# ray-project/kuberay

Measured on NVIDIA H100. Metric: reconciles/sec over 10k RayCluster x 100 pods (batched reconcilePods + status roll-up), higher is better.
Workload: dtype u32

## Files before the change

kuberay_b200/csrc/kr_bucket2.cuh:

```cuda
#pragma once

#include "kr_decide.cuh"

namespace kr {

__device__ __forceinline__ uint32_t inc_epoch_of(const ScratchDev &sc) { return __ldcg(&sc.inc[KR_INC_EPOCH]) + 1u; }

#ifndef KR_D2WARPS
#define KR_D2WARPS 8
#endif
static constexpr int kD2Warps = KR_D2WARPS;
#define KR_ROW_UNHEALTHY (1u << 13)
#define KR_ROW_FRESH (1u << 14)
#define KR_LG_OWNED (1u << 31)

__device__ __forceinline__ uint4 *large_slot(const ScratchDev &sc, uint32_t c, uint32_t rank) {
  if (!sc.lg) return nullptr;
  const uint4 l = __ldcg(&sc.lg[c]);
  const uint32_t j = rank - sc.bucket_stride;
  return j < l.y ? sc.region + l.x + j : nullptr;
}
__device__ __forceinline__ uint4 *rec_slot(const ScratchDev &sc, uint32_t c, uint32_t rank) {
  return rank < sc.bucket_stride ? sc.bucket + (size_t)c * sc.bucket_stride + rank : large_slot(sc, c, rank);
}


template <int kItems>
__global__ void __launch_bounds__(kSortThreads) k_match2(SnapDev s, ScratchDev sc, ResDev r, Sizes n, int has_wtd) {
  KR_TL(1);
  extern __shared__ uint32_t sm_bits[];
  __shared__ uint32_t s_orph[kSortThreads / 32];
  const uint32_t tile = blockIdx.x;
  const uint32_t warp = threadIdx.x >> 5, lane = threadIdx.x & 31;
  const uint32_t base = tile * (kSortThreads * kItems) + warp * (32 * kItems) + lane;
  uint32_t ns[kItems], cn[kItems], gn[kItems], nm[kItems], pk[kItems], ri[kItems];
#pragma unroll
  for (int it = 0; it < kItems; it++) {
    const uint32_t p = base + it * 32;
    const bool v = p < n.n_pods;
    ns[it] = v ? __ldg(&s.p_ns_id[p]) : 0u; cn[it] = v ? __ldg(&s.p_cluster_name_id[p]) : 0u;
    gn[it] = v ? __ldg(&s.p_group_name_id[p]) : 0u; nm[it] = v ? __ldg(&s.p_name_id[p]) : 0u;
    pk[it] = v ? __ldg(&s.p_packed[p]) : 0u; ri[it] = v ? (uint32_t)__ldg(&s.p_replica_index[p]) : 0u;
  }
  pdl_wait(); pdl_trigger();
  uint32_t pi[kItems];
  uint4 sl[kItems];
#pragma unroll
  for (int it = 0; it < kItems; it++) {
    pi[it] = hash_pair(ns[it], cn[it]) & sc.cl_mask;
    sl[it] = __ldg(&sc.cl_slots[pi[it]]);
  }
  if (has_wtd) {
    const uint32_t words = (sc.wt_bits_mask + 1) >> 5;
    for (uint32_t i = threadIdx.x; i < words; i += kSortThreads) sm_bits[i] = __ldcg(&sc.wt_bits[i]);
    __syncthreads();
  }
  uint32_t orphans = 0;
  uint32_t cidx[kItems], roww[kItems];
#pragma unroll
  for (int it = 0; it < kItems; it++) {
    const uint32_t p = base + it * 32;
    const bool v = p < n.n_pods;
    uint32_t c = n.n_clusters, cflags = 0, gname0 = 0;
    if (cn[it] != 0) {
      uint4 q = sl[it];
      uint32_t i = pi[it];
      while (true) {
        if (q.x == cn[it] && q.y == ns[it]) { c = q.w >> 2; cflags = q.w & 3u; gname0 = q.z; break; }
        if (q.x == KR_EMPTY32 && q.y == KR_EMPTY32) break;
        i = (i + 1) & sc.cl_mask;
        q = __ldg(&sc.cl_slots[i]);
      }
    }
    const bool matched = v && c < n.n_clusters;
    uint32_t slot = KR_ROW_NO_GROUP, g0 = 0xFFFFFFFFu;
    if (matched && gn[it] != 0) {
      if (gname0 == gn[it]) slot = 0;
      else if (cflags & KR_CL_MULTI) {
        const uint4 rec = __ldg(&sc.cl_rec[c]);
        g0 = rec.x;
        for (uint32_t gi = 1; gi < rec.y; gi++)
          if (__ldg(&s.g_name_id[g0 + gi]) == gn[it]) { slot = gi; break; }
      }
    }
    uint32_t flags = pk[it] & (0x7FFu | KR_PP_TOMBSTONE);
    if (should_delete(pk[it])) flags |= KR_ROW_UNHEALTHY;
    if (has_wtd && v) {
      const uint32_t hk = hash_pair(ns[it], nm[it]);
      const uint32_t h2 = bloom2(hk);
      if ((sm_bits[(hk & sc.wt_bits_mask) >> 5] & (1u << (hk & 31))) && (sm_bits[(h2 & sc.wt_bits_mask) >> 5] & (1u << (h2 & 31)))) {
        const uint64_t k = key2(ns[it], nm[it]);
        uint32_t i = hk & sc.wt_mask;
        uint64_t kk = __ldg(&sc.wt_keys[i]);
        while (kk != KR_EMPTY64) {
          if (kk == k) {
            for (uint32_t e = sc.wt_head[i]; e != KR_EMPTY32; e = sc.wt_next[e]) {
// ... 139 lines not shown
      if ((((labelled | noname) >> k) & 1u) && (pw[k] & KR_ROW_WTD_OWN)) {
        const uint32_t r = ((noname >> k) & 1u) ? r_empty : rep[k];
        if (r != KR_MH_NONE) atomicOr(&s_rep[r], KR_MHF_WTD);
      }
    }
    __syncwarp();
    int32_t n_del = 0;
#pragma unroll
    for (int k = 0; k < K; k++) {
      const bool hit = ((labelled >> k) & 1u) && (s_rep[rep[k]] & KR_MHF_WTD);
      if (hit && act[k] == KR_ACT_KEEP) act[k] = KR_ACT_DELETE_MH_WTD;
      n_del += __popc(__ballot_sync(0xFFFFFFFFu, hit));
    }
    gr.flags |= KR_GR_WTD_EXECUTED;
    if (n_del > 0) { gr.flags |= KR_GR_ABORTED; err_arg = n_del; return KR_ERR_MH_WTD; }
  }
  int32_t running = 0;
  for (uint32_t r = lane; r < n_rep; r += 32) running += (s_rep[r] & KR_MHF_DELETED) ? 0 : 1;
  running = __reduce_add_sync(0xFFFFFFFFu, running);
#pragma unroll
  for (int k = 0; k < K; k++) if (((heads >> k) & 1u) && !(s_rep[rep[k]] & KR_MHF_DELETED)) mh_head |= 1u << k;
  gr.n_running = running;
  if (expected % H != 0) { gr.flags |= KR_GR_ABORTED; err_arg = expected; return KR_ERR_MH_NOT_MULTIPLE; }
  const int32_t to_create = expected / H - running;
  gr.diff = to_create;
  if (to_create > 0) gr.n_create = (uint32_t)to_create;
  else if (to_create < 0) {
    if (delete_allowed) {
      const int32_t remove = -to_create;
      int32_t seen = 0;
      for (uint32_t b = 0; b < n_rep && seen < remove; b += 32) {
        const uint32_t r = b + lane;
        const bool ok = r < n_rep && !(s_rep[r] & KR_MHF_DELETED);
        const uint32_t bal = __ballot_sync(0xFFFFFFFFu, ok);
        if (ok && seen + (int32_t)__popc(bal & lt) < remove) s_rep[r] |= KR_MHF_SCALE;
        seen += __popc(bal);
      }
      __syncwarp();
#pragma unroll
      for (int k = 0; k < K; k++) if (((labelled >> k) & 1u) && (s_rep[rep[k]] & KR_MHF_SCALE)) act[k] = KR_ACT_DELETE_MH_SCALE_DOWN;
    } else gr.flags |= KR_GR_RANDOM_DELETE_OFF;
  }
  return KR_ERR_NONE;
}

template <int K, bool kInc = false, bool kMH = false>
__global__ void __launch_bounds__(kD2Warps * 32, (K <= 4 && !kMH ? 32 : 16) / kD2Warps) k_decide2(Decide2Args a) {
  const int phase = kInc ? 2 : a.phase;
  KR_TL(phase ? 12 : 3);
  __shared__ int32_t s_acc[kD2Warps][3][KR_SMEM_GROUPS];
  __shared__ int32_t s_mode[kD2Warps][kMH ? 4 : 3][KR_SMEM_GROUPS];
  __shared__ uint32_t s_list[kD2Warps][32 * K];
  __shared__ uint32_t s_bits[kD2Warps][32];
  const SnapDev &s = a.s;
  const uint32_t warp = threadIdx.x >> 5, lane = threadIdx.x & 31;
  const uint32_t lt = lanemask_lt();
  const uint32_t S = a.sc.bucket_stride;
  uint32_t c = blockIdx.x * kD2Warps + warp;
  bool mine = phase == 0 && c < a.n.n_clusters;
  RecordCI ci{mine ? __ldg(&a.sc.cl_in[32 * (size_t)c + lane]) : 0u};
  pdl_wait(); pdl_trigger();
  if (phase == 1) {
    mine = c < a.r.totals[4];
    if (mine) { c = a.sc.deferred_list[c]; ci.word = __ldg(&a.sc.cl_in[32 * (size_t)c + lane]); }
  } else if (kInc) {
    mine = c < __ldcg(&a.sc.inc[KR_INC_DIRTY]) && !__ldcg(&a.sc.inc[KR_INC_VOID]) && !__ldcg(&a.sc.inc[KR_INC_STRUCTURAL]);
    if (mine) {
      c = a.sc.dirty_list[c];
      ci.word = __ldcg(&a.sc.cl_in[32 * (size_t)c + lane]);
    }
  }
  if (KR_ATTEMPT_VOID(a.r.totals)) mine = false;
  if (ci.group_cnt() > KR_SMEM_GROUPS) mine = false;
  if (kInc && !mine) return;
  uint4 *bucket = a.sc.bucket + (size_t)(mine ? c : 0) * S;
  uint4 dyn = make_uint4(0, 0, 0, 0);
  uint4 recs[K] = {};
  if (mine) {
    dyn = __ldcg(&a.sc.cl_dyn[c]);
#pragma unroll
    for (int k = 0; k < K; k++) if ((uint32_t)(k * 32) + lane < S) recs[k] = __ldcg(&bucket[k * 32 + lane]);
  }
  uint32_t P = dyn.x;
  if (P > S) { mine = false; P = 0; }
  if (kInc) {
    const uint32_t epoch = inc_epoch_of(a.sc);
    const bool lost = dyn.y == epoch;
    uint32_t kept = 0, head_min = 0xFFFFFFFFu;
#pragma unroll
    for (int k = 0; k < K; k++) {
      const uint32_t j = k * 32 + lane;
      bool keep = mine && j < P;
      const bool fresh = keep && (recs[k].y & KR_ROW_FRESH);
      if (keep && lost && !fresh) keep = __ldcg(&a.sc.stamp[recs[k].x]) != epoch;
      const uint32_t bal = __ballot_sync(0xFFFFFFFFu, keep);
      if (keep) {
        uint4 rec = recs[k];
        rec.y &= ~KR_ROW_FRESH;
        const uint32_t to = kept + __popc(bal & lt);
        if (fresh || to != j) { bucket[to] = rec; if (to != j) a.sc.pos[rec.x] = to; }
        if (pp_node_type(rec.y & 0xFFFFu) == KR_NT_HEAD) head_min = min(head_min, rec.x);
      }
      kept += __popc(bal);
    }
    head_min = __reduce_min_sync(0xFFFFFFFFu, head_min);
    __syncwarp();
    unsigned long long raw = 0;
    if (mine) {
      if (lane == 0 && head_min != 0xFFFFFFFFu) raw = ~(((unsigned long long)head_min << 32) | (uint32_t)(aux_lookup(a.sc, head_min) + 1));
      raw = __shfl_sync(0xFFFFFFFFu, raw, 0);
      P = kept;
      dyn = make_uint4(kept, 0u, (uint32_t)raw, (uint32_t)(raw >> 32));
      if (lane == 0) a.sc.cl_dyn[c] = dyn;
#pragma unroll
      for (int k = 0; k < K; k++) if ((uint32_t)(k * 32) + lane < kept) recs[k] = __ldcg(&bucket[k * 32 + lane]);
    }
  }
  const uint32_t cf = ci.flags(), G = ci.group_cnt(), g0 = ci.group_off();
  const uint8_t suspend_status = ci.suspend_status(), ext_err = ci.ext_err_kind(), old_prov = ci.cond_status(KR_COND_PROVISIONED);
  const bool gate = a.f.gate_status_conditions != 0;
  uint32_t old_create = 0;
  if (kInc && mine) {
    for (uint32_t gi = lane; gi < G; gi += 32) old_create += a.r.groups[g0 + gi].n_create;
    old_create = __reduce_add_sync(0xFFFFFFFFu, old_create);
  }
  uint32_t head_pod = 0xFFFFFFFFu;
  int32_t head_aux = -1;
  {
    const unsigned long long raw = ((unsigned long long)dyn.w << 32) | dyn.z;
    if (mine && raw != 0) { const unsigned long long key = ~raw; head_pod = (uint32_t)(key >> 32); head_aux = (int32_t)(uint32_t)key - 1; }
  }
  uint8_t h_ver = KR_VER_EMPTY, h_ast = KR_ANNOT_EMPTY;
  if (head_aux >= 0 && (cf & KR_CF_UPGRADE_RECREATE)) { h_ver = s.h_version_state[head_aux]; h_ast = s.h_annot_state[head_aux]; }
  uint32_t pidx[K], pw[K], ridx[K], act[K];
  uint32_t head_pos = 0xFFFFFFFFu, head_name = 0, head_flags = 0;
#pragma unroll
  for (int k = 0; k < K; k++) {
    const uint32_t i = k * 32 + lane;
    const bool valid = i < P;
    pidx[k] = valid ? recs[k].x : 0xFFFFFFFFu; pw[k] = valid ? recs[k].y : (KR_ROW_NO_GROUP << 16); ridx[k] = valid ? recs[k].z : 0u; act[k] = KR_ACT_KEEP;
    const uint32_t hit = __ballot_sync(0xFFFFFFFFu, valid && recs[k].x == head_pod);
    if (hit) {
      const int src = __ffs(hit) - 1;
      head_pos = k * 32 + src;
      head_name = __shfl_sync(0xFFFFFFFFu, recs[k].w, src); head_flags = __shfl_sync(0xFFFFFFFFu, recs[k].y, src) & 0xFFFFu;
    }
  }
  (void)head_pos;
  int32_t *acc_list = s_acc[warp][0], *acc_unh = s_acc[warp][1], *acc_wtd = s_acc[warp][2];
  int32_t *g_mode = s_mode[warp][0], *g_prefix = s_mode[warp][1], *g_ncreate = s_mode[warp][2], *g_mh_running = s_mode[warp][kMH ? 3 : 2];
  uint32_t mh_head = 0;
  if (lane < KR_SMEM_GROUPS) { acc_list[lane] = 0; acc_unh[lane] = 0; acc_wtd[lane] = 0; g_mode[lane] = GM_UNPROCESSED; g_prefix[lane] = 0; g_ncreate[lane] = 0; }
  __syncwarp();

  int32_t ready = 0, available = 0, n_heads = 0, n0_list = 0, n0_unh = 0, n0_wtd = 0;
  bool all_running = P > 0;
  const uint32_t nchunks = (P + 31) / 32;
#pragma unroll
  for (int k = 0; k < K; k++) {
    if ((uint32_t)k >= nchunks) break;
    const bool valid = (uint32_t)(k * 32) + lane < P;
    const uint32_t w = pw[k], fl = w & 0xFFFFu, slot = valid ? (w >> 16) : KR_ROW_NO_GROUP;
    const uint32_t nt = pp_node_type(fl), ph = pp_phase(fl), rd = pp_ready(fl);
    const bool w_run = valid && nt == KR_NT_WORKER && ph == KR_PHASE_RUNNING;
    available += __popc(__ballot_sync(0xFFFFFFFFu, w_run));
    ready += __popc(__ballot_sync(0xFFFFFFFFu, w_run && rd == KR_COND_TRUE));
    const bool not_ok = valid && (ph != KR_PHASE_RUNNING || rd == KR_COND_FALSE || rd == KR_COND_UNKNOWN);
    if (__any_sync(0xFFFFFFFFu, not_ok)) all_running = false;
    n_heads += __popc(__ballot_sync(0xFFFFFFFFu, valid && nt == KR_NT_HEAD));
    if (G == 1) {
      const bool in0 = slot == 0;
      n0_list += __popc(__ballot_sync(0xFFFFFFFFu, in0));
      n0_unh += __popc(__ballot_sync(0xFFFFFFFFu, in0 && (fl & KR_ROW_UNHEALTHY)));
      n0_wtd += __popc(__ballot_sync(0xFFFFFFFFu, in0 && (fl & KR_ROW_WTD_OWN)));
      continue;
    }
    const uint32_t gkey = (slot < G) ? slot : KR_ROW_NO_GROUP;
    const uint32_t peers = __match_any_sync(0xFFFFFFFFu, gkey);
    if (gkey != KR_ROW_NO_GROUP) {
      const uint32_t ub = __ballot_sync(peers, (fl & KR_ROW_UNHEALTHY) != 0);
      const uint32_t wb = __ballot_sync(peers, (fl & KR_ROW_WTD_OWN) != 0);
      if ((peers & lt) == 0) {
        acc_list[gkey] += __popc(peers);
        acc_unh[gkey] += __popc(ub & peers);
        acc_wtd[gkey] += __popc(wb & peers);
      }
    }
    __syncwarp();
  }
  if (G == 1) { if (lane == 0) { acc_list[0] = n0_list; acc_unh[0] = n0_unh; acc_wtd[0] = n0_wtd; } __syncwarp(); }

  kr_cluster_result cr;
  {
    uint32_t *z = reinterpret_cast<uint32_t *>(&cr);
#pragma unroll
    for (int k = 0; k < (int)(sizeof(cr) / 4); k++) z[k] = 0;
  }
  cr.head_pod_idx = -1; cr.stop_after_group = -1;
  uint8_t all_action = KR_ACT_KEEP;
  bool head_delete = false, run_groups = false, deferred = false, any_prefix = false;
  uint32_t n_create_cluster = 0;
  if (mine) {
    if (cf & KR_CF_SKIP) {
      cr.path = KR_PATH_SKIPPED;
    } else if (ext_err != KR_EXT_ERR_NONE) {
      cr.path = KR_PATH_SKIPPED;
      cr.err_kind = ext_err == KR_EXT_ERR_STATUS_ONLY_NIL ? KR_ERR_NONE : KR_ERR_EXTERNAL;
    } else if (suspend_status == KR_SUSPEND_SUSPENDING || (!gate && (cf & KR_CF_SUSPEND))) {
      cr.path = KR_PATH_SUSPENDING_DELETE_ALL; all_action = KR_ACT_DELETE_ALL_SUSPEND;
    } else if (gate && (suspend_status == KR_SUSPEND_SUSPENDED || (cf & KR_CF_SUSPEND))) {
      cr.path = KR_PATH_SUSPENDED_NOOP;
    } else {
      bool recreate = false;
      if ((cf & KR_CF_UPGRADE_RECREATE) && n_heads > 0) {
        const int32_t aux = head_aux;
        const uint8_t ver = h_ver, ast = h_ast;
        if (ver == KR_VER_DIFFERENT) cr.head_update_annotations = 1;
        else if (ast == KR_ANNOT_OTHER) recreate = true;
        else if (ast == KR_ANNOT_HASH32 && !a.f.skip_hash) {
          if (phase == 0 && !a.spin_hash) {
            deferred = true;
            if (lane == 0) a.sc.deferred_list[atomicAdd(&a.r.totals[4], 1u)] = c;
          } else {
            const uint8_t *ah = s.h_annot_hash + 32 * (size_t)aux;
            const uint32_t *hw = reinterpret_cast<const uint32_t *>(a.r.hash + 32 * (size_t)c);
            if (phase == 0) {
              if (lane == 0) {
                const volatile uint32_t *w7 = hw + 7;
                uint32_t it = 0;
                while (*w7 == 0u && it < 40000u) { __nanosleep(100); it++; }
                if (*w7 == 0u) atomicOr(&a.r.totals[3], KR_TOTALS_HASH_WAIT);
              }
              __syncwarp();
              __threadfence();
            }
            const uint32_t word = __ldcg(&hw[lane >> 2]);
            recreate = __any_sync(0xFFFFFFFFu, ah[lane] != (uint8_t)(word >> (8 * (lane & 3))));
          }
        }
      }
      if (recreate) {
        cr.path = KR_PATH_RECREATE_DELETE_ALL; all_action = KR_ACT_DELETE_ALL_RECREATE;
      } else {
        cr.path = KR_PATH_NORMAL;
        if (!(cf & KR_CF_HEAD_EXPECT_OK)) { cr.head_action = KR_HEAD_EXPECT_PENDING; run_groups = true; }
        else if (n_heads == 1) {
          if (head_flags & KR_ROW_UNHEALTHY) { cr.head_action = KR_HEAD_DELETE; cr.err_kind = KR_ERR_HEAD_DELETED; head_delete = true; }
          else run_groups = true;
        } else if (n_heads == 0) {
          if (old_prov == KR_COND_TRUE && (cf & KR_CF_SKIP_HEAD_RESTART)) cr.head_action = KR_HEAD_SKIP_RESTART;
          else { cr.head_action = KR_HEAD_CREATE; run_groups = true; }
// ... 21 lines not shown
        } else {
          const int32_t expected = desired_replicas(g_rep, g_mn, g_mx, hosts, gf);
          const int32_t n_list = acc_list[gi], n_unh = acc_unh[gi], n_wtd = acc_wtd[gi];
          gr.expected = expected; gr.n_list = n_list;
          if (gf & KR_GF_SUSPEND) { gr.flags |= KR_GR_SUSPENDED; mode = GM_SUSPENDED; }
          else if (kMH && hosts > 1 && a.f.gate_multihost_indexing) {
            gr.flags |= KR_GR_MULTIHOST; mode = GM_MULTIHOST;
            int32_t earg = 0;
            const int ek = decide_multihost2<K>(s, gi, expected, hosts, !autoscaling || a.f.env_random_pod_delete, LDG(s.g_wtd_cnt[g]), pidx, pw, act, mh_head,
                                                s_list[warp], gr, earg, lane);
            if (ek != KR_ERR_NONE) { cr.err_kind = (uint8_t)ek; cr.err_arg = earg; abort_here = true; }
            if (lane == 0) g_mh_running[gi] = gr.n_running;
          }
          else if (n_unh > 0) {
            gr.n_unhealthy = n_unh; gr.flags |= KR_GR_ABORTED; mode = GM_UNHEALTHY;
            cr.err_kind = KR_ERR_UNHEALTHY_WORKERS; cr.err_arg = n_unh; abort_here = true;
          } else {
            gr.flags |= KR_GR_WTD_EXECUTED; mode = GM_NORMAL;
            const int32_t running = n_list - n_wtd;
            const int32_t diff = expected - running;
            gr.n_running = running; gr.diff = diff;
            if (diff > 0) gr.n_create = (uint32_t)diff;
            else if (diff < 0) {
              if (!autoscaling || a.f.env_random_pod_delete) {
                const long long remove = -(long long)diff;
                if (remove > running) {
                  prefix = running; gr.flags |= KR_GR_ABORTED;
                  cr.err_kind = KR_ERR_NEGATIVE_EXPECTED; cr.err_arg = expected; abort_here = true;
                } else prefix = (int32_t)remove;
              } else gr.flags |= KR_GR_RANDOM_DELETE_OFF;
            }
          }
        }
        any_prefix |= prefix > 0;
        n_create_cluster += gr.n_create;
        __syncwarp();
        if (lane == 0) {
          g_mode[gi] = mode; g_prefix[gi] = prefix; g_ncreate[gi] = (int32_t)gr.n_create;
          a.r.groups[g] = gr;
        }
        if (abort_here) { cr.stop_after_group = (int32_t)gi; break; }
      }
    }
    {
      const int32_t reached = ((cf & KR_CF_SKIP) || !run_groups) ? 0 : (cr.stop_after_group == (int32_t)G ? (int32_t)G : cr.stop_after_group + 1);
      for (uint32_t gi = reached + lane; gi < G; gi += 32) {
        kr_group_result z; z.expected = 0; z.n_list = 0; z.n_unhealthy = 0; z.n_running = 0; z.diff = 0; z.n_create = 0; z.create_off = 0; z.flags = 0;
        a.r.groups[g0 + gi] = z;
      }
    }
  }
  __syncwarp();

  uint32_t cand = 0;
  if (mine) {
#pragma unroll
    for (int k = 0; k < K; k++) {
      if ((uint32_t)k >= nchunks) break;
      const bool valid = (uint32_t)(k * 32) + lane < P;
      const uint32_t w = pw[k], fl = w & 0xFFFFu;
      const uint32_t gkey = (valid && run_groups && (w >> 16) < G) ? (w >> 16) : KR_ROW_NO_GROUP;
      const int32_t mode = (gkey != KR_ROW_NO_GROUP) ? g_mode[gkey] : GM_UNPROCESSED;
      uint32_t ac = KR_ACT_KEEP;
      if (all_action != KR_ACT_KEEP) ac = valid ? all_action : (uint32_t)KR_ACT_KEEP;
      else if (head_delete) { if (valid && pidx[k] == head_pod) ac = KR_ACT_DELETE_HEAD; }
      else if (mode == GM_SUSPENDED) ac = KR_ACT_DELETE_GROUP_SUSPEND;
      else if (kMH && mode == GM_MULTIHOST) ac = act[k];
      else if (mode == GM_UNHEALTHY) { if (fl & KR_ROW_UNHEALTHY) ac = KR_ACT_DELETE_UNHEALTHY; }
      else if (mode == GM_NORMAL) {
        if (fl & KR_ROW_WTD_OWN) ac = KR_ACT_DELETE_WTD;
        else cand |= 1u << k;
      }
      act[k] = ac;
    }
    if (any_prefix) {
      for (uint32_t gi = 0; gi < G; gi++) {
        const int32_t pre = g_prefix[gi];
        if (pre <= 0) continue;
        if (pre <= 8) {
          for (int32_t it = 0; it < pre; it++) {
            uint32_t m = 0xFFFFFFFFu;
#pragma unroll
            for (int k = 0; k < K; k++)
              if (((cand >> k) & 1u) && (pw[k] >> 16) == gi && act[k] == KR_ACT_KEEP) m = min(m, pidx[k]);
            const uint32_t wm = __reduce_min_sync(0xFFFFFFFFu, m);
            if (wm == 0xFFFFFFFFu) break;
#pragma unroll
            for (int k = 0; k < K; k++)
              if (((cand >> k) & 1u) && pidx[k] == wm) act[k] = KR_ACT_DELETE_RANDOM;
          }
        } else {
          uint32_t nc = 0;
#pragma unroll
          for (int k = 0; k < K; k++) {
            const bool isc = ((cand >> k) & 1u) && (pw[k] >> 16) == gi;
            const uint32_t bal = __ballot_sync(0xFFFFFFFFu, isc);
            if (isc) s_list[warp][nc + __popc(bal & lt)] = pidx[k];
            nc += __popc(bal);
          }
          __syncwarp();
#pragma unroll
          for (int k = 0; k < K; k++) {
            const bool isc = ((cand >> k) & 1u) && (pw[k] >> 16) == gi;
            if (!__any_sync(0xFFFFFFFFu, isc)) continue;
            uint32_t rank = 0;
            for (uint32_t i = 0; i < nc; i++) rank += s_list[warp][i] < pidx[k] ? 1u : 0u;
            if (isc && (int32_t)rank < pre) act[k] = KR_ACT_DELETE_RANDOM;
          }
          __syncwarp();
        }
      }
    }
  }
  uint32_t n_act = 0;
  uint32_t arank[K];
#pragma unroll
  for (int k = 0; k < K; k++) {
    arank[k] = 0;
    const bool isa = act[k] != KR_ACT_KEEP;
    const uint32_t bal = __ballot_sync(0xFFFFFFFFu, isa);
    if (isa) s_list[warp][n_act + __popc(bal & lt)] = pidx[k];
    n_act += __popc(bal);
  }
  __syncwarp();
  if (n_act > 1) {
#pragma unroll
    for (int k = 0; k < K; k++) {
      const bool isa = act[k] != KR_ACT_KEEP;
      if (!__any_sync(0xFFFFFFFFu, isa)) continue;
      uint32_t rank = 0;
      for (uint32_t i = 0; i < n_act; i++) rank += s_list[warp][i] < pidx[k] ? 1u : 0u;
      arank[k] = rank;
    }
  }

  if (!(cf & KR_CF_SKIP))
    status_rollup(a.s, a.f, ci, cr, P, (uint32_t)n_heads, n_heads > 0 ? (int32_t)head_pod : -1, head_aux, head_name, ready, available, all_running);
  if (mine && lane == 0) a.r.clusters[c] = cr;

  const uint32_t slots = deferred ? P : n_act;
  uint32_t act_off = 0, create_off = 0;
  if (phase == 0) {
    unsigned long long base = 0;
    if (mine && lane == 0) {
      if (slots | n_create_cluster) base = atomicAdd(reinterpret_cast<unsigned long long *>(&a.r.totals[8]), ((unsigned long long)n_create_cluster << 32) | slots);
      if (n_act) atomicAdd(&a.r.totals[2], n_act);
      if (n_create_cluster) atomicAdd(&a.r.totals[6], n_create_cluster);
    }
    base = __shfl_sync(0xFFFFFFFFu, base, 0);
    act_off = (uint32_t)base; create_off = (uint32_t)(base >> 32);
    if (mine && lane == 0) {
      a.r.act_start[c] = act_off; a.r.act_cnt[c] = n_act;
      if (deferred) a.sc.cact[c] = n_create_cluster;
      a.sc.act_res[c] = slots; a.sc.cre_res[c] = n_create_cluster;
    }
  } else if (kInc) {
    unsigned long long base = 0;
    uint32_t need = 0;
    if (mine && lane == 0) {
      const uint32_t old_act = a.r.act_cnt[c];
      need = (n_act > a.sc.act_res[c] ? 1u : 0u) | (n_create_cluster > a.sc.cre_res[c] ? 2u : 0u);
      if (need) base = atomicAdd(reinterpret_cast<unsigned long long *>(&a.r.totals[8]), ((unsigned long long)((need & 2u) ? n_create_cluster : 0u) << 32) | ((need & 1u) ? n_act : 0u));
      if ((need & 1u) && (uint64_t)(uint32_t)base + n_act > a.n.n_pods) a.sc.inc[KR_INC_VOID] = 1u;
      if ((need & 2u) && (uint64_t)(uint32_t)(base >> 32) + n_create_cluster > a.create_cap) a.sc.inc[KR_INC_VOID] = 1u;
      if (n_act != old_act) atomicAdd(&a.r.totals[2], n_act - old_act);
      if (n_create_cluster != old_create) atomicAdd(&a.r.totals[6], n_create_cluster - old_create);
    }
    base = __shfl_sync(0xFFFFFFFFu, base, 0); need = __shfl_sync(0xFFFFFFFFu, need, 0);
    if (mine) {
      act_off = (need & 1u) ? (uint32_t)base : a.r.act_start[c];
      create_off = (need & 2u) ? (uint32_t)(base >> 32) : (G ? a.sc.gcreate[g0] : 0u);
      if ((need & 1u) && (uint64_t)act_off + n_act > a.n.n_pods) mine = false;
      if ((need & 2u) && (uint64_t)create_off + n_create_cluster > a.create_cap) mine = false;
      if (mine && lane == 0) {
        a.r.act_start[c] = act_off; a.r.act_cnt[c] = n_act;
        if (need & 1u) a.sc.act_res[c] = n_act;
        if (need & 2u) a.sc.cre_res[c] = n_create_cluster;
      }
    }
  } else if (mine) {
    act_off = a.r.act_start[c];
    if (lane == 0) {
      const uint32_t old_act = a.r.act_cnt[c], old_create = a.sc.cact[c];
      a.r.act_cnt[c] = n_act;
      if (n_act != old_act) atomicAdd(&a.r.totals[2], n_act - old_act);
      if (n_create_cluster != old_create) atomicAdd(&a.r.totals[6], n_create_cluster - old_create);
    }
  }
  if (!mine) return;
#pragma unroll
  for (int k = 0; k < K; k++)
    if (act[k] != KR_ACT_KEEP) { a.r.act_pod_idx[act_off + arank[k]] = pidx[k]; a.r.act_code[act_off + arank[k]] = (uint8_t)act[k]; }
  if (phase == 1 || n_create_cluster) {
    uint32_t off = create_off;
    for (uint32_t gi = 0; gi < G; gi++) {
      const uint32_t g = g0 + gi;
      const uint32_t want = (uint32_t)g_ncreate[gi];
      if (phase == 1) {
        off = a.sc.gcreate[g];
      }
      if (lane == 0) { a.r.groups[g].create_off = off; if (phase != 1) a.sc.gcreate[g] = off; }
      if (want == 0) continue;
      if ((uint64_t)off + want > a.create_cap) { off += want; continue; }
      int32_t *out = a.r.create_idx + off;
      if (!a.f.gate_multihost_indexing) {
        for (uint32_t k2 = lane; k2 < want; k2 += 32) out[k2] = -1;
      } else {
        const bool mh = kMH && g_mode[gi] == GM_MULTIHOST;
        const uint64_t bound = (uint64_t)(mh ? g_mh_running[gi] : acc_list[gi] - acc_wtd[gi]) + want;
        uint32_t written = 0;
        for (uint64_t w0 = 0; w0 < bound && written < want; w0 += 1024) {
          s_bits[warp][lane] = 0;
          __syncwarp();
#pragma unroll
          for (int k = 0; k < K; k++) {
            if ((pw[k] >> 16) == gi && (pw[k] & KR_PP_HAS_REPLICA_IDX) && (mh ? ((mh_head >> k) & 1u) != 0 : (act[k] == KR_ACT_KEEP && pidx[k] != 0xFFFFFFFFu))) {
              const int32_t idx = (int32_t)ridx[k];
              if (idx >= 0 && (uint64_t)idx >= w0 && (uint64_t)idx < w0 + 1024 && (uint64_t)idx < bound)
                atomicOr(&s_bits[warp][(idx - w0) >> 5], 1u << ((idx - w0) & 31));
            }
          }
          __syncwarp();
          const uint32_t word = s_bits[warp][lane];
          const uint64_t wbase = w0 + 32ull * lane;
          uint32_t freeb = ~word;
          if (wbase >= bound) freeb = 0;
          else if (bound - wbase < 32) freeb &= (1u << (uint32_t)(bound - wbase)) - 1;
          const uint32_t cnt = __popc(freeb);
          uint32_t x = cnt;
#pragma unroll
          for (int d = 1; d < 32; d <<= 1) { const uint32_t y = __shfl_up_sync(0xFFFFFFFFu, x, d); if (lane >= (uint32_t)d) x += y; }
          uint32_t pos = written + x - cnt;
          while (freeb && pos < want) {
            const uint32_t bit = __ffs(freeb) - 1;
            freeb &= freeb - 1;
            out[pos++] = (int32_t)(wbase + bit);
          }
          written += __shfl_sync(0xFFFFFFFFu, x, 31);
          __syncwarp();
        }
      }
      off += want;
    }
  } else if (G) {
    for (uint32_t gi = lane; gi < G; gi += 32) { a.r.groups[g0 + gi].create_off = create_off; a.sc.gcreate[g0 + gi] = create_off; }
  }
  if (kInc) {
    __syncwarp();
    stage_cluster(a, blockIdx.x * kD2Warps + warp, c, act_off, n_act, g0, G, lane);
  }
}

}
```

kuberay_b200/csrc/kr_engine.cu:

```cuda
#include <cuda_runtime.h>

#include <algorithm>
#include <chrono>
#include <cstdarg>
#include <cstdio>
#include <cstdlib>
#include <cstring>
#include <string>
#include <thread>
#include <vector>

#include "kr_kernels.cuh"
#include "kr_incr.cuh"
#include "kr_large.cuh"
#include "kr_huge.cuh"

using namespace kr;

int kr_specjson_emit_string(const uint8_t *spec_json, uint64_t len, bool muted, long max_groups, std::string &out, long *n_groups);

namespace {

constexpr size_t kAlign = 256;
inline size_t align_up(size_t x, size_t a = kAlign) { return (x + a - 1) / a * a; }
// ... 409 lines not shown
  std::vector<uint32_t> list, huge;
  std::vector<uint4> tiles;
  for (size_t i = 0; i < e->large_rows.size(); i++) {
    const uint32_t c = e->large_rows[i], cap = e->large_reg[i].y;
    if (!is_huge(e->bstride, cap)) { list.push_back(c); continue; }
    huge.push_back(c);
    const uint32_t nt = huge_tile_count(e->bstride, cap), first = (uint32_t)tiles.size();
    for (uint32_t t = 0; t < nt; t++) tiles.push_back(make_uint4(c, t * kHugeTile, first, nt));
  }
  if (e->wide_on)
    for (uint32_t c : e->wide_rows) if (!std::binary_search(e->large_rows.begin(), e->large_rows.end(), c)) list.push_back(c);
  const uint32_t n_lsort = (uint32_t)list.size();
  list.insert(list.end(), huge.begin(), huge.end());
  if (tiles.size() > e->huge_tiles) return fail(e, KR_E_STATE, "internal: %zu huge-cluster tiles, room for %zu", tiles.size(), e->huge_tiles);
  if ((uint32_t)list.size() != e->n_large || n_lsort != e->n_lsort || (uint32_t)tiles.size() != e->n_tiles) e->gvalid = false;
  e->n_large = (uint32_t)list.size(); e->n_lsort = n_lsort; e->n_tiles = (uint32_t)tiles.size();
  if (list.empty()) return KR_OK;
  const uint32_t Nc = e->sizes.n_clusters;
  std::vector<uint4> lg(Nc, make_uint4(0, 0, 0, 0));
  for (size_t i = 0; i < e->large_rows.size(); i++) lg[e->large_rows[i]] = make_uint4(e->large_reg[i].x, e->large_reg[i].y, 0, 0);
  CK(cudaStreamSynchronize(e->sm));
  e->h_lg.swap(lg); e->h_lg_list.swap(list); e->h_tiles.swap(tiles);
  CK(cudaMemcpyAsync(e->d_lg, e->h_lg.data(), 16 * (size_t)Nc, cudaMemcpyHostToDevice, e->sm));
  CK(cudaMemcpyAsync(e->d_lg + align_up(16 * (size_t)e->cfg.max_clusters), e->h_lg_list.data(), 4 * e->h_lg_list.size(), cudaMemcpyHostToDevice, e->sm));
  if (!e->h_tiles.empty()) CK(cudaMemcpyAsync(e->d_huge, e->h_tiles.data(), 16 * e->h_tiles.size(), cudaMemcpyHostToDevice, e->sm));
  return KR_OK;
}

int launch_pass(kr_engine *e, const kr_flags &f, bool profile, bool capturing = false) {
  const kr_sizes &n = e->sizes;
  SnapDev s;
  bind_in(e->il, e->d_in, &s);
  ResDev r = bind_out(e->ol, e->d_out);
  ScratchDev sc = bind_scratch(e->sl, e->d_scratch);
  const uint32_t *lg_list = bind_large(e, sc);
  const HugeDev hd = bind_huge(e);
  Sizes z{n.n_clusters, n.n_groups, n.n_wtd, n.n_pods, n.n_heads, n.n_jobs};
  cudaStream_t M = e->sm, H = profile ? e->sm : e->sh;
  int k = 0;
  auto mark = [&](const char *name) {
    if (profile && k < KR_MAX_KERNEL_TIMES) { e->prof.kernel_name[k] = name; cudaEventRecord(e->ev_k[k], M); }
    k++;
  };
  e->prof.n_kernels = 0;

  const bool do_hash = !f.skip_hash && n.n_clusters > 0;
  const unsigned wflag = capturing ? cudaEventWaitExternal : cudaEventWaitDefault;
  const bool bucket = !e->no_bucket && !f.fetch_pod_lists && e->bstride != 0 && !e->force_radix && (e->snap_max_groups <= KR_SMEM_GROUPS || e->wide_on) &&
                      (size_t)n.n_clusters * e->bstride <= e->sl.bucket_entries;
  const bool spin = bucket && !profile && do_hash && e->hash_spin && e->n_recreate > 0;
  auto launch_hash = [&]() {
    const uint32_t ngroups = (n.n_clusters + 31) / 32;
    if (ngroups <= (uint32_t)e->sm_count * 4) {
      const uint32_t G = std::min<uint32_t>(ngroups, (uint32_t)e->sm_count * 2);
      k_hash3<1, 0><<<G, 64, sizeof(H3Smem), H>>>(s.json, s.c_json_off, s.c_json_len, e->d_order, n.n_clusters, r.hash);
    } else {
      uint32_t blocks = std::min<uint32_t>((n.n_clusters + 127) / 128, (uint32_t)e->sm_count * e->hash_ctas_per_sm);
      k_hash2<4, 1><<<blocks, 128, 0, H>>>(s.json, s.c_json_off, s.c_json_len, e->d_order, n.n_clusters, r.hash, 1u);
    }
  };
  auto start_hash_stream = [&]() -> int {
    if (profile) return KR_OK;
    CK(cudaEventRecord(e->ev_fork, M)); CK(cudaStreamWaitEvent(H, e->ev_fork, 0));
    CK(cudaStreamWaitEvent(H, e->ev_json, wflag));
    if (do_hash && spin && n.n_clusters) CK(cudaMemsetAsync(r.hash, 0, 32 * (size_t)n.n_clusters, H));
    if (do_hash) { launch_hash(); k++; }
    else if (n.n_clusters) CK(cudaMemsetAsync(r.hash, 0, 32 * (size_t)n.n_clusters, H));
    CK(cudaEventRecord(e->ev_hash, H));
    return KR_OK;
  };
  { int rc = start_hash_stream(); if (rc) return rc; }

  e->ran_bucket = bucket;
  sc.bucket_stride = e->bstride;
  const bool pdl = !profile && e->use_pdl;
  bool fuse_place_done = false;
  bool creates_after_kernel = false;
  {
    ClearArgs ca{};
    ca.ptr[0] = reinterpret_cast<uint32_t *>(e->d_scratch); ca.words[0] = (uint32_t)(e->sl.ff_total / 4); ca.value[0] = 0xFFFFFFFFu;
    ca.ptr[1] = r.wtd_pod_idx; ca.words[1] = n.n_wtd; ca.value[1] = 0xFFFFFFFFu;
    ca.ptr[2] = r.totals; ca.words[2] = 64; ca.value[2] = 0;
    ca.ptr[3] = sc.ccount; ca.words[3] = (uint32_t)((e->sl.cstart - e->sl.ccount) / 4); ca.value[3] = 0;
    mark("k_clear");
    k_clear<<<e->sm_count * 2, 256, 0, M>>>(ca);
  }
  CK(cudaStreamWaitEvent(M, e->ev_cols, wflag));
  {
    uint32_t items = n.n_clusters + n.n_groups + n.n_heads;
    if (items) { mark("k_build_tables"); k_build_tables<<<(items + 255) / 256, 256, 0, M>>>(s, sc, r, z); }
  }
  if (bucket) {
    e->ran_fast = false;
    const uint32_t mtiles = e->sl.mtiles;
    if (n.n_pods) {
      mark("k_match2");
      CK(launch_pdl(k_match2<kMatchItems>, dim3(mtiles), dim3(kSortThreads), n.n_wtd ? e->sl.wt_bits_n / 8 : 0, M, pdl, s, sc, r, z, n.n_wtd ? 1 : 0));
    }
    Decide2Args da{s, sc, r, z, f, IncStage{}, e->cfg.max_creates, spin ? 1 : 0, 0};
    const bool mh = e->snap_has_mh && f.gate_multihost_indexing;
    auto launch_decide2 = [&](dim3 grid, bool with_pdl) -> cudaError_t {
      const dim3 block(kD2Warps * 32);
      if (e->bstride <= 64) return launch_pdl(mh ? k_decide2<2, false, true> : k_decide2<2>, grid, block, 0, M, with_pdl, da);
      if (e->bstride <= 128) return launch_pdl(mh ? k_decide2<4, false, true> : k_decide2<4>, grid, block, 0, M, with_pdl, da);
      return launch_pdl(mh ? k_decide2<8, false, true> : k_decide2<8>, grid, block, 0, M, with_pdl, da);
    };
    if (n.n_clusters) {
      mark("k_decide2");
      CK(launch_decide2(dim3((n.n_clusters + kD2Warps - 1) / kD2Warps), pdl && n.n_pods != 0));
    } else CK(cudaMemsetAsync(r.act_start, 0, 4, M));
    if (n.n_jobs) { mark("k_jobs"); k_jobs<<<(n.n_jobs + 255) / 256, 256, 0, M>>>(s, sc, r, z); }
    const bool large = e->n_large && sc.lg && n.n_clusters;
    if (large && e->n_lsort) { mark("k_large_sort"); k_large_sort<false><<<e->n_lsort, kLargeSortThreads, 0, M>>>(da, lg_list); }
    if (large && e->n_tiles) {
      mark("k_huge_tiles"); k_huge_tiles<false><<<e->n_tiles, kHugeThreads, 0, M>>>(da, hd);
      mark("k_huge_merge"); k_huge_merge<false><<<e->n_tiles, kHugeThreads, 0, M>>>(da, hd);
    }
    if (profile) {
      if (do_hash) { mark("k_hash"); launch_hash(); }
      else if (n.n_clusters) CK(cudaMemsetAsync(r.hash, 0, 32 * (size_t)n.n_clusters, M));
    } else {
      CK(cudaStreamWaitEvent(M, e->ev_hash, 0));
    }
    if (large) { mark("k_decide_large"); k_decide_large<false><<<e->n_large, kLargeDecideThreads, 0, M>>>(da, lg_list); }
    if (e->n_recreate > 0 && do_hash && !spin) {
      da.phase = 1;
      mark("k_decide2_phase1");
      CK(launch_decide2(dim3((e->n_recreate + kD2Warps - 1) / kD2Warps), false));
    }
  } else {
  const uint32_t ntiles = e->sl.ntiles;
  const bool fast = !e->force_radix;
  e->ran_fast = fast;
  const uint32_t *sorted_keys = sc.keys[0];
  if (n.n_pods && fast) {
    mark("k_match");
    const uint32_t mtiles = e->sl.mtiles;
    CK(launch_pdl(k_match<true, kMatchItems>, dim3(mtiles), dim3(kSortThreads), 0, M, pdl, s, sc, r, z, n.n_wtd ? 1 : 0));
    const bool fuse_place = !e->no_fuse && (uint64_t)n.n_clusters + 2 + mtiles <= kFusedMaxCounters;
    if (fuse_place) {
      fuse_place_done = true;
      mark("k_place_fused");
      size_t smem = 4 * ((size_t)n.n_clusters + 2 + mtiles);
      CK(launch_pdl(k_place_fused, dim3(e->sm_count * e->place_ctas), dim3(1024), smem, M, pdl, (const uint32_t *)sc.keys[0], (const uint32_t *)sc.keys[1], (const uint32_t *)sc.ccount, sc.cstart,
                    (const uint32_t *)sc.tile_orph, sc.vals[0], n.n_pods, n.n_clusters, mtiles, r.totals));
    } else {
    mark("k_scan_counts");
    const uint32_t nch_c = (n.n_clusters + 1 + kScanChunk - 1) / kScanChunk, nch_t = (mtiles + kScanChunk - 1) / kScanChunk;
    k_scan_counts<<<nch_c + nch_t, 1024, 0, M>>>(sc.ccount, sc.cstart, n.n_clusters + 1, nch_c, sc.tile_orph, mtiles, sc.chain, r.totals);
    mark("k_place");
    k_place<<<(n.n_pods + 1023) / 1024, 256, 0, M>>>(sc.keys[0], sc.keys[1], sc.cstart, sc.tile_orph, sc.vals[0], n.n_pods, n.n_clusters);
    }
  } else if (n.n_pods) {
    uint32_t bits = 1;
    while ((1ull << bits) <= n.n_clusters) bits++;
    const int passes = (int)((bits + kRadixBits - 1) / kRadixBits);
    mark("k_match");
    k_match<false, kSortItems><<<ntiles, kSortThreads, 0, M>>>(s, sc, r, z, n.n_wtd ? 1 : 0);
    int cur = 0;
    for (int p = 0; p < passes; p++) {
      if (p > 0) { mark("k_hist"); k_hist<<<ntiles, kSortThreads, 0, M>>>(sc.keys[cur], sc.hist, n.n_pods, p * kRadixBits); }
      mark("k_scan_rows");
// ... 1288 lines not shown
```

kuberay_b200/csrc/kr_match.cuh:

```cuda
#pragma once

#include "kr_common.cuh"

namespace kr {

struct ClearArgs { uint32_t *ptr[4]; uint32_t words[4]; uint32_t value[4]; };
__global__ void __launch_bounds__(256) k_clear(ClearArgs a) {
  KR_TL(9);
  const uint32_t stride = gridDim.x * blockDim.x, t0 = blockIdx.x * blockDim.x + threadIdx.x;
#pragma unroll
  for (int r = 0; r < 4; r++) {
    uint32_t *p = a.ptr[r];
    const uint32_t v = a.value[r], nw = a.words[r];
    uint4 *p4 = reinterpret_cast<uint4 *>(p);
    for (uint32_t i = t0; i < nw / 4; i += stride) p4[i] = make_uint4(v, v, v, v);
    for (uint32_t i = (nw & ~3u) + t0; i < nw; i += stride) p[i] = v;
  }
}

__device__ __forceinline__ void write_cl_in(const SnapDev &s, const ScratchDev &sc, uint32_t t, uint32_t g0, uint32_t G) {
  uint32_t *ci = sc.cl_in + 32 * (size_t)t;
  const uint8_t *cs = s.c_old_cond_status + 5 * (size_t)t, *cv = s.c_old_cond_variant + 5 * (size_t)t;
  uint4 w0, w1;
  w0.x = s.c_flags[t]; w0.y = g0; w0.z = G;
  w0.w = s.c_suspend_status[t] | ((uint32_t)s.c_ext_err_kind[t] << 8) | ((uint32_t)s.c_old_state[t] << 16) | ((uint32_t)s.c_svc_count[t] << 24);
  w1.x = s.c_svc_ip_kind[t] | ((uint32_t)cs[0] << 8) | ((uint32_t)cs[1] << 16) | ((uint32_t)cs[2] << 24);
  w1.y = cs[3] | ((uint32_t)cs[4] << 8) | ((uint32_t)cv[0] << 16) | ((uint32_t)cv[1] << 24);
  w1.z = cv[2] | ((uint32_t)cv[3] << 8) | ((uint32_t)cv[4] << 16);
  w1.w = s.c_ext_err_msg_id[t];
  uint4 *o = reinterpret_cast<uint4 *>(ci);
  o[0] = w0; o[1] = w1;
  const int32_t *oc = s.c_old_counts + 5 * (size_t)t;
  o[2] = make_uint4((uint32_t)oc[0], (uint32_t)oc[1], (uint32_t)oc[2], (uint32_t)oc[3]);
  o[3] = make_uint4((uint32_t)oc[4], s.c_old_cond_reason_id[t], s.c_old_cond_msg_id[2 * (size_t)t], s.c_old_cond_msg_id[2 * (size_t)t + 1]);
  const uint32_t *oh = s.c_old_head_ids + 4 * (size_t)t;
  o[4] = make_uint4(oh[0], oh[1], oh[2], oh[3]);
  uint4 w5 = make_uint4(s.c_svc_ip_id[t], s.c_svc_name_id[t], 0, 0), w6 = make_uint4(0, 0, 0, 0);
  if (G) { w5.z = s.g_flags[g0]; w5.w = (uint32_t)s.g_replicas[g0]; w6.x = (uint32_t)s.g_min[g0]; w6.y = (uint32_t)s.g_max[g0]; w6.z = (uint32_t)s.g_num_hosts[g0]; }
  o[5] = w5; o[6] = w6; o[7] = make_uint4(0, 0, 0, 0);
}

__device__ __forceinline__ void wt_insert_group(const SnapDev &s, const ScratchDev &sc, uint32_t t) {
  uint32_t c = s.g_cluster_idx[t];
  uint32_t ns = s.c_ns_id[c];
  uint32_t off = s.g_wtd_off[t], cnt = s.g_wtd_cnt[t];
  for (uint32_t w = 0; w < cnt; w++) {
    uint32_t e = off + w;
    uint64_t k = key2(ns, s.w_name_id[e]);
    const uint32_t hk = hash_pair(ns, s.w_name_id[e]);
    atomicOr(&sc.wt_bits[(hk & sc.wt_bits_mask) >> 5], 1u << (hk & 31));
    { const uint32_t h2 = bloom2(hk); atomicOr(&sc.wt_bits[(h2 & sc.wt_bits_mask) >> 5], 1u << (h2 & 31)); }
    uint32_t i = hk & sc.wt_mask;
    while (true) {
      unsigned long long prev = atomicCAS((unsigned long long *)&sc.wt_keys[i], KR_EMPTY64, k);
      if (prev == KR_EMPTY64 || prev == k) {
        uint32_t old = atomicExch(&sc.wt_head[i], e);
        sc.wt_next[e] = old;
        break;
      }
      i = (i + 1) & sc.wt_mask;
    }
  }
}


__global__ void __launch_bounds__(256) k_build_tables(SnapDev s, ScratchDev sc, ResDev r, Sizes n) {
  KR_TL(0);
  pdl_trigger();
  uint32_t t = blockIdx.x * blockDim.x + threadIdx.x;
  if (t == 0) {
    sc.inc[KR_INC_TOUCHED] = 0; sc.inc[KR_INC_DIRTY] = 0; sc.inc[KR_INC_STRUCTURAL] = 0; sc.inc[KR_INC_HEADS] = 0; sc.inc[KR_INC_VOID] = 0; sc.inc[KR_INC_GROUPS] = 0; sc.inc[KR_INC_LSEG] = 0;
    sc.inc[KR_INC_EPOCH] += 1u;
  }
  if (t < n.n_clusters) {
    uint32_t ns = s.c_ns_id[t], name = s.c_name_id[t];
    uint32_t i = hash_pair(ns, name) & sc.cl_mask;
    unsigned long long *slots = reinterpret_cast<unsigned long long *>(sc.cl_slots);
    const unsigned long long kk = ((unsigned long long)ns << 32) | name;
    uint32_t g0 = s.c_group_off[t], G = s.c_group_cnt[t], mh = 0;
    for (uint32_t gi = 0; gi < G; gi++) mh |= (s.g_num_hosts[g0 + gi] > 1) ? 1u : 0u;
    const uint32_t gname0 = G ? s.g_name_id[g0] : 0u;
    const unsigned long long payload = ((unsigned long long)((t << 2) | (G > 1 ? KR_CL_MULTI : 0u) | mh) << 32) | gname0;
    while (true) {
      unsigned long long prev = atomicCAS(&slots[2 * (size_t)i], KR_EMPTY64, kk);
      if (prev == KR_EMPTY64 || prev == kk) { atomicMin(&slots[2 * (size_t)i + 1], payload); break; }
      i = (i + 1) & sc.cl_mask;
    }
    sc.cl_rec[t] = make_uint4(g0, G, gname0, mh);
    write_cl_in(s, sc, t, g0, G);
    return;
  }
  t -= n.n_clusters;
  if (t < n.n_groups) {
    wt_insert_group(s, sc, t);
    return;
  }
  t -= n.n_groups;
  if (t < n.n_heads) {
    uint32_t p = s.h_pod_idx[t];
    uint32_t i = mix32(p) & sc.aux_mask;
    while (true) {
      uint32_t prev = atomicCAS(&sc.aux_keys[i], KR_EMPTY32, p);
      if (prev == KR_EMPTY32 || prev == p) { atomicMin(&sc.aux_vals[i], t); break; }
      i = (i + 1) & sc.aux_mask;
    }
  }
}

__device__ __forceinline__ int32_t aux_lookup(const ScratchDev &sc, uint32_t p) {
  uint32_t i = mix32(p) & sc.aux_mask;
  while (true) {
    uint32_t k = sc.aux_keys[i];
    if (k == p) return (int32_t)sc.aux_vals[i];
    if (k == KR_EMPTY32) return -1;
    i = (i + 1) & sc.aux_mask;
  }
}


template <bool kFast, int kItems>
__global__ void __launch_bounds__(kSortThreads) k_match(SnapDev s, ScratchDev sc, ResDev r, Sizes n, int has_wtd) {
  KR_TL(1);
  __shared__ uint32_t s_hist[kRadix];
  pdl_wait(); pdl_trigger();
  const uint32_t tile = blockIdx.x, ntiles = gridDim.x;
  const uint32_t warp = threadIdx.x >> 5, lane = threadIdx.x & 31;
  if (!kFast) { s_hist[threadIdx.x] = 0; __syncthreads(); }
  const uint32_t base = tile * (kSortThreads * kItems) + warp * (32 * kItems) + lane;
  uint32_t ns[kItems], cn[kItems], gn[kItems], nm[kItems], pk[kItems], rn[kItems], ri[kItems];
#pragma unroll
  for (int it = 0; it < kItems; it++) {
    uint32_t p = base + it * 32;
    bool v = p < n.n_pods;
    ns[it] = v ? __ldg(&s.p_ns_id[p]) : 0u; cn[it] = v ? __ldg(&s.p_cluster_name_id[p]) : 0u;
    gn[it] = v ? __ldg(&s.p_group_name_id[p]) : 0u; nm[it] = v ? __ldg(&s.p_name_id[p]) : 0u;
    pk[it] = v ? __ldg(&s.p_packed[p]) : 0u; ri[it] = v ? (uint32_t)__ldg(&s.p_replica_index[p]) : 0u;
    rn[it] = v ? __ldg(&s.p_replica_name_id[p]) : 0u;
  }
  uint32_t c[kItems], pi[kItems];
  uint4 sl[kItems];
#pragma unroll
  for (int it = 0; it < kItems; it++) {
// ... 93 lines not shown
```

Before: 82.73 million.

## Overlap prologue work via PDL and move cluster-input packing into match kernel

The per-cluster input packing moves from k_build_tables into k_match2, placed before the PDL wait so it overlaps the previous kernel. k_clear and k_build_tables now take part in programmatic dependent launch, with k_build_tables loading its cluster fields before waiting. k_decide2 splits bucket records into separate registers, builds the cluster result in shared memory and writes it lane-parallel, moves the status roll-up earlier, and rereads replica indices from global memory to reduce register pressure. The hash launch now uses one block per group with no cap. These changes add cross-kernel ordering risk around cl_in being written in match and read in decide, and make decide depend on match running even when there are no pods.

```diff
diff --git a/kuberay_b200/csrc/kr_bucket2.cuh b/kuberay_b200/csrc/kr_bucket2.cuh
--- a/kuberay_b200/csrc/kr_bucket2.cuh
+++ b/kuberay_b200/csrc/kr_bucket2.cuh
@@ -42,6 +42,8 @@
     gn[it] = v ? __ldg(&s.p_group_name_id[p]) : 0u; nm[it] = v ? __ldg(&s.p_name_id[p]) : 0u;
     pk[it] = v ? __ldg(&s.p_packed[p]) : 0u; ri[it] = v ? (uint32_t)__ldg(&s.p_replica_index[p]) : 0u;
   }
+  for (uint32_t c = tile * kSortThreads + threadIdx.x; c < n.n_clusters; c += gridDim.x * kSortThreads)
+    write_cl_in(s, sc, c, s.c_group_off[c], s.c_group_cnt[c]);
   pdl_wait(); pdl_trigger();
   uint32_t pi[kItems];
   uint4 sl[kItems];
@@ -287,15 +289,18 @@
   __shared__ int32_t s_mode[kD2Warps][kMH ? 4 : 3][KR_SMEM_GROUPS];
   __shared__ uint32_t s_list[kD2Warps][32 * K];
   __shared__ uint32_t s_bits[kD2Warps][32];
+  __shared__ kr_cluster_result s_cr[kD2Warps];
   const SnapDev &s = a.s;
   const uint32_t warp = threadIdx.x >> 5, lane = threadIdx.x & 31;
   const uint32_t lt = lanemask_lt();
   const uint32_t S = a.sc.bucket_stride;
   uint32_t c = blockIdx.x * kD2Warps + warp;
   bool mine = phase == 0 && c < a.n.n_clusters;
-  RecordCI ci{mine ? __ldg(&a.sc.cl_in[32 * (size_t)c + lane]) : 0u};
+  RecordCI ci{0u};
   pdl_wait(); pdl_trigger();
-  if (phase == 1) {
+  if (phase == 0) {
+    if (mine) ci.word = __ldcg(&a.sc.cl_in[32 * (size_t)c + lane]);
+  } else if (phase == 1) {
     mine = c < a.r.totals[4];
     if (mine) { c = a.sc.deferred_list[c]; ci.word = __ldg(&a.sc.cl_in[32 * (size_t)c + lane]); }
   } else if (kInc) {
@@ -310,11 +315,17 @@
   if (kInc && !mine) return;
   uint4 *bucket = a.sc.bucket + (size_t)(mine ? c : 0) * S;
   uint4 dyn = make_uint4(0, 0, 0, 0);
-  uint4 recs[K] = {};
+  uint32_t pidx[K], pw[K], ridx[K], pname[K], act[K];
+#pragma unroll
+  for (int k = 0; k < K; k++) { pidx[k] = 0u; pw[k] = 0u; ridx[k] = 0u; pname[k] = 0u; act[k] = KR_ACT_KEEP; }
+  auto load_bucket = [&](uint32_t n) {
+#pragma unroll
+    for (int k = 0; k < K; k++)
+      if ((uint32_t)(k * 32) + lane < n) { const uint4 q = __ldcg(&bucket[k * 32 + lane]); pidx[k] = q.x; pw[k] = q.y; ridx[k] = q.z; pname[k] = q.w; }
+  };
   if (mine) {
     dyn = __ldcg(&a.sc.cl_dyn[c]);
-#pragma unroll
-    for (int k = 0; k < K; k++) if ((uint32_t)(k * 32) + lane < S) recs[k] = __ldcg(&bucket[k * 32 + lane]);
+    load_bucket(S);
   }
   uint32_t P = dyn.x;
   if (P > S) { mine = false; P = 0; }
@@ -326,12 +337,11 @@
     for (int k = 0; k < K; k++) {
       const uint32_t j = k * 32 + lane;
       bool keep = mine && j < P;
-      const bool fresh = keep && (recs[k].y & KR_ROW_FRESH);
-      if (keep && lost && !fresh) keep = __ldcg(&a.sc.stamp[recs[k].x]) != epoch;
+      const bool fresh = keep && (pw[k] & KR_ROW_FRESH);
+      if (keep && lost && !fresh) keep = __ldcg(&a.sc.stamp[pidx[k]]) != epoch;
       const uint32_t bal = __ballot_sync(0xFFFFFFFFu, keep);
       if (keep) {
-        uint4 rec = recs[k];
-        rec.y &= ~KR_ROW_FRESH;
+        const uint4 rec = make_uint4(pidx[k], pw[k] & ~KR_ROW_FRESH, ridx[k], pname[k]);
         const uint32_t to = kept + __popc(bal & lt);
         if (fresh || to != j) { bucket[to] = rec; if (to != j) a.sc.pos[rec.x] = to; }
         if (pp_node_type(rec.y & 0xFFFFu) == KR_NT_HEAD) head_min = min(head_min, rec.x);
@@ -347,8 +357,7 @@
       P = kept;
       dyn = make_uint4(kept, 0u, (uint32_t)raw, (uint32_t)(raw >> 32));
       if (lane == 0) a.sc.cl_dyn[c] = dyn;
-#pragma unroll
-      for (int k = 0; k < K; k++) if ((uint32_t)(k * 32) + lane < kept) recs[k] = __ldcg(&bucket[k * 32 + lane]);
+      load_bucket(kept);
     }
   }
   const uint32_t cf = ci.flags(), G = ci.group_cnt(), g0 = ci.group_off();
@@ -367,21 +376,17 @@
   }
   uint8_t h_ver = KR_VER_EMPTY, h_ast = KR_ANNOT_EMPTY;
   if (head_aux >= 0 && (cf & KR_CF_UPGRADE_RECREATE)) { h_ver = s.h_version_state[head_aux]; h_ast = s.h_annot_state[head_aux]; }
-  uint32_t pidx[K], pw[K], ridx[K], act[K];
-  uint32_t head_pos = 0xFFFFFFFFu, head_name = 0, head_flags = 0;
+  uint32_t head_name = 0, head_flags = 0;
 #pragma unroll
   for (int k = 0; k < K; k++) {
-    const uint32_t i = k * 32 + lane;
-    const bool valid = i < P;
-    pidx[k] = valid ? recs[k].x : 0xFFFFFFFFu; pw[k] = valid ? recs[k].y : (KR_ROW_NO_GROUP << 16); ridx[k] = valid ? recs[k].z : 0u; act[k] = KR_ACT_KEEP;
-    const uint32_t hit = __ballot_sync(0xFFFFFFFFu, valid && recs[k].x == head_pod);
+    const bool valid = (uint32_t)(k * 32) + lane < P;
+    if (!valid) { pidx[k] = 0xFFFFFFFFu; pw[k] = KR_ROW_NO_GROUP << 16; }
+    const uint32_t hit = __ballot_sync(0xFFFFFFFFu, valid && pidx[k] == head_pod);
     if (hit) {
       const int src = __ffs(hit) - 1;
-      head_pos = k * 32 + src;
-      head_name = __shfl_sync(0xFFFFFFFFu, recs[k].w, src); head_flags = __shfl_sync(0xFFFFFFFFu, recs[k].y, src) & 0xFFFFu;
-    }
-  }
-  (void)head_pos;
+      head_name = __shfl_sync(0xFFFFFFFFu, pname[k], src); head_flags = __shfl_sync(0xFFFFFFFFu, pw[k], src) & 0xFFFFu;
+    }
+  }
   int32_t *acc_list = s_acc[warp][0], *acc_unh = s_acc[warp][1], *acc_wtd = s_acc[warp][2];
   int32_t *g_mode = s_mode[warp][0], *g_prefix = s_mode[warp][1], *g_ncreate = s_mode[warp][2], *g_mh_running = s_mode[warp][kMH ? 3 : 2];
   uint32_t mh_head = 0;
@@ -425,13 +430,13 @@
   }
   if (G == 1) { if (lane == 0) { acc_list[0] = n0_list; acc_unh[0] = n0_unh; acc_wtd[0] = n0_wtd; } __syncwarp(); }
 
-  kr_cluster_result cr;
-  {
-    uint32_t *z = reinterpret_cast<uint32_t *>(&cr);
-#pragma unroll
-    for (int k = 0; k < (int)(sizeof(cr) / 4); k++) z[k] = 0;
-  }
-  cr.head_pod_idx = -1; cr.stop_after_group = -1;
+  static_assert(sizeof(kr_cluster_result) % 4 == 0 && sizeof(kr_cluster_result) / 4 <= 32, "record size");
+  constexpr uint32_t kCrWords = sizeof(kr_cluster_result) / 4;
+  kr_cluster_result &cr = s_cr[warp];
+  if (lane < kCrWords)
+    reinterpret_cast<uint32_t *>(&cr)[lane] =
+        (lane == offsetof(kr_cluster_result, head_pod_idx) / 4 || lane == offsetof(kr_cluster_result, stop_after_group) / 4) ? 0xFFFFFFFFu : 0u;
+  __syncwarp();
   uint8_t all_action = KR_ACT_KEEP;
   bool head_delete = false, run_groups = false, deferred = false, any_prefix = false;
   uint32_t n_create_cluster = 0;
@@ -559,6 +564,11 @@
   }
   __syncwarp();
 
+  if (!(cf & KR_CF_SKIP))
+    status_rollup(a.s, a.f, ci, cr, P, (uint32_t)n_heads, n_heads > 0 ? (int32_t)head_pod : -1, head_aux, head_name, ready, available, all_running);
+  __syncwarp();
+  if (mine && lane < kCrWords) reinterpret_cast<uint32_t *>(&a.r.clusters[c])[lane] = reinterpret_cast<const uint32_t *>(&cr)[lane];
+
   uint32_t cand = 0;
   if (mine) {
 #pragma unroll
@@ -641,10 +651,6 @@
     }
   }
 
-  if (!(cf & KR_CF_SKIP))
-    status_rollup(a.s, a.f, ci, cr, P, (uint32_t)n_heads, n_heads > 0 ? (int32_t)head_pod : -1, head_aux, head_name, ready, available, all_running);
-  if (mine && lane == 0) a.r.clusters[c] = cr;
-
   const uint32_t slots = deferred ? P : n_act;
   uint32_t act_off = 0, create_off = 0;
   if (phase == 0) {
@@ -722,7 +728,7 @@
 #pragma unroll
           for (int k = 0; k < K; k++) {
             if ((pw[k] >> 16) == gi && (pw[k] & KR_PP_HAS_REPLICA_IDX) && (mh ? ((mh_head >> k) & 1u) != 0 : (act[k] == KR_ACT_KEEP && pidx[k] != 0xFFFFFFFFu))) {
-              const int32_t idx = (int32_t)ridx[k];
+              const int32_t idx = (int32_t)__ldcg(&a.sc.bucket[(size_t)c * S + k * 32 + lane].z);
               if (idx >= 0 && (uint64_t)idx >= w0 && (uint64_t)idx < w0 + 1024 && (uint64_t)idx < bound)
                 atomicOr(&s_bits[warp][(idx - w0) >> 5], 1u << ((idx - w0) & 31));
             }
diff --git a/kuberay_b200/csrc/kr_engine.cu b/kuberay_b200/csrc/kr_engine.cu
--- a/kuberay_b200/csrc/kr_engine.cu
+++ b/kuberay_b200/csrc/kr_engine.cu
@@ -485,7 +485,7 @@
   auto launch_hash = [&]() {
     const uint32_t ngroups = (n.n_clusters + 31) / 32;
     if (ngroups <= (uint32_t)e->sm_count * 4) {
-      const uint32_t G = std::min<uint32_t>(ngroups, (uint32_t)e->sm_count * 2);
+      const uint32_t G = ngroups;
       k_hash3<1, 0><<<G, 64, sizeof(H3Smem), H>>>(s.json, s.c_json_off, s.c_json_len, e->d_order, n.n_clusters, r.hash);
     } else {
       uint32_t blocks = std::min<uint32_t>((n.n_clusters + 127) / 128, (uint32_t)e->sm_count * e->hash_ctas_per_sm);
@@ -509,6 +509,7 @@
   const bool pdl = !profile && e->use_pdl;
   bool fuse_place_done = false;
   bool creates_after_kernel = false;
+  CK(cudaStreamWaitEvent(M, e->ev_cols, wflag));
   {
     ClearArgs ca{};
     ca.ptr[0] = reinterpret_cast<uint32_t *>(e->d_scratch); ca.words[0] = (uint32_t)(e->sl.ff_total / 4); ca.value[0] = 0xFFFFFFFFu;
@@ -518,15 +519,14 @@
     mark("k_clear");
     k_clear<<<e->sm_count * 2, 256, 0, M>>>(ca);
   }
-  CK(cudaStreamWaitEvent(M, e->ev_cols, wflag));
   {
     uint32_t items = n.n_clusters + n.n_groups + n.n_heads;
-    if (items) { mark("k_build_tables"); k_build_tables<<<(items + 255) / 256, 256, 0, M>>>(s, sc, r, z); }
+    if (items) { mark("k_build_tables"); CK(launch_pdl(k_build_tables, dim3((items + 255) / 256), dim3(256), 0, M, pdl, s, sc, r, z)); }
   }
   if (bucket) {
     e->ran_fast = false;
     const uint32_t mtiles = e->sl.mtiles;
-    if (n.n_pods) {
+    if (n.n_pods || n.n_clusters) {
       mark("k_match2");
       CK(launch_pdl(k_match2<kMatchItems>, dim3(mtiles), dim3(kSortThreads), n.n_wtd ? e->sl.wt_bits_n / 8 : 0, M, pdl, s, sc, r, z, n.n_wtd ? 1 : 0));
     }
@@ -540,7 +540,7 @@
     };
     if (n.n_clusters) {
       mark("k_decide2");
-      CK(launch_decide2(dim3((n.n_clusters + kD2Warps - 1) / kD2Warps), pdl && n.n_pods != 0));
+      CK(launch_decide2(dim3((n.n_clusters + kD2Warps - 1) / kD2Warps), pdl));
     } else CK(cudaMemsetAsync(r.act_start, 0, 4, M));
     if (n.n_jobs) { mark("k_jobs"); k_jobs<<<(n.n_jobs + 255) / 256, 256, 0, M>>>(s, sc, r, z); }
     const bool large = e->n_large && sc.lg && n.n_clusters;
diff --git a/kuberay_b200/csrc/kr_match.cuh b/kuberay_b200/csrc/kr_match.cuh
--- a/kuberay_b200/csrc/kr_match.cuh
+++ b/kuberay_b200/csrc/kr_match.cuh
@@ -7,6 +7,7 @@
 struct ClearArgs { uint32_t *ptr[4]; uint32_t words[4]; uint32_t value[4]; };
 __global__ void __launch_bounds__(256) k_clear(ClearArgs a) {
   KR_TL(9);
+  pdl_trigger();
   const uint32_t stride = gridDim.x * blockDim.x, t0 = blockIdx.x * blockDim.x + threadIdx.x;
 #pragma unroll
   for (int r = 0; r < 4; r++) {
@@ -68,18 +69,22 @@
   KR_TL(0);
   pdl_trigger();
   uint32_t t = blockIdx.x * blockDim.x + threadIdx.x;
+  const bool cl = t < n.n_clusters;
+  uint32_t ns = 0, name = 0, g0 = 0, G = 0, mh = 0, gname0 = 0;
+  if (cl) {
+    ns = s.c_ns_id[t]; name = s.c_name_id[t]; g0 = s.c_group_off[t]; G = s.c_group_cnt[t];
+    for (uint32_t gi = 0; gi < G; gi++) mh |= (s.g_num_hosts[g0 + gi] > 1) ? 1u : 0u;
+    gname0 = G ? s.g_name_id[g0] : 0u;
+  }
+  pdl_wait();
   if (t == 0) {
     sc.inc[KR_INC_TOUCHED] = 0; sc.inc[KR_INC_DIRTY] = 0; sc.inc[KR_INC_STRUCTURAL] = 0; sc.inc[KR_INC_HEADS] = 0; sc.inc[KR_INC_VOID] = 0; sc.inc[KR_INC_GROUPS] = 0; sc.inc[KR_INC_LSEG] = 0;
     sc.inc[KR_INC_EPOCH] += 1u;
   }
-  if (t < n.n_clusters) {
-    uint32_t ns = s.c_ns_id[t], name = s.c_name_id[t];
+  if (cl) {
     uint32_t i = hash_pair(ns, name) & sc.cl_mask;
     unsigned long long *slots = reinterpret_cast<unsigned long long *>(sc.cl_slots);
     const unsigned long long kk = ((unsigned long long)ns << 32) | name;
-    uint32_t g0 = s.c_group_off[t], G = s.c_group_cnt[t], mh = 0;
-    for (uint32_t gi = 0; gi < G; gi++) mh |= (s.g_num_hosts[g0 + gi] > 1) ? 1u : 0u;
-    const uint32_t gname0 = G ? s.g_name_id[g0] : 0u;
     const unsigned long long payload = ((unsigned long long)((t << 2) | (G > 1 ? KR_CL_MULTI : 0u) | mh) << 32) | gname0;
     while (true) {
       unsigned long long prev = atomicCAS(&slots[2 * (size_t)i], KR_EMPTY64, kk);
@@ -87,7 +92,6 @@
       i = (i + 1) & sc.cl_mask;
     }
     sc.cl_rec[t] = make_uint4(g0, G, gname0, mh);
-    write_cl_in(s, sc, t, g0, G);
     return;
   }
   t -= n.n_clusters;
```

New measurement: 87.51 million (median of 6 runs). 1.06x the previous value.
